# wangheda/youtube-8m

Measured on AMD Instinct MI355X. Metric: training videos/sec, higher is better.
Workload: dtype f32; 1 GPU; BASELINE configs[3]: LstmModel (2 x BasicLSTMCell(1024), dynamic_rnn over F=300) on raw uint8 [B,300,1152] frames + MoeModel head (2 mixtures, V=4716), fp32 training step (fwd+bwd+clip+Adam); per_gpu_batch=128, global_batch=128, frames=300, parallelism=dp1, params=113902808

## Files before the change

### include/yt8m_hip.h

```cpp
#ifndef YT8M_HIP_H
#define YT8M_HIP_H
#include <stdint.h>

#ifdef __cplusplus
extern "C" {
#endif

typedef void* yt8m_stream_t;

enum yt8m_status { YT8M_OK = 0, YT8M_E_BADARG = -1, YT8M_E_SHAPE = -2, YT8M_E_HIP = -3, YT8M_E_RCCL = -4 };
enum yt8m_label_dtype { YT8M_LABEL_U8 = 0, YT8M_LABEL_F32 = 1 };

int yt8m_abi_version(void);
const char* yt8m_last_error(void);
const char* yt8m_built_arch(void);

int yt8m_prof_enable(int on);
int yt8m_prof_reset(void);
int yt8m_prof_get(int family, int64_t* launches, double* total_ms);
int yt8m_prof_get_flops(int family, double* flops);
int yt8m_prof_get_bytes(int family, double* bytes);

int yt8m_probe_mfma_f32(int iters, int blocks, float* sink, yt8m_stream_t stream);
int yt8m_probe_mfma_bf16(int iters, int blocks, int random_operands, float* sink, yt8m_stream_t stream);
// ... 10 lines not shown
                          const float* A, int64_t lda, int64_t strideA, const float* B, int64_t ldb, int64_t strideB,
                          float* C, int64_t ldc, int64_t strideC, float beta, int64_t batch, yt8m_stream_t stream);

typedef struct yt8m_gemm_problem {
  int64_t M, N, K;
  const void* A; int64_t lda;
  const void* B; int64_t ldb;
  float* C; int64_t ldc;
  const float* bias;
  float beta;
} yt8m_gemm_problem;
int64_t yt8m_gemm_workspace_bytes(void);
int yt8m_gemm_f32_grouped(int transA, int transB, int nprob, const yt8m_gemm_problem* probs, void* workspace,
                          int64_t workspace_bytes, yt8m_stream_t stream);
int yt8m_gemm_bf16_nt_grouped(int nprob, const yt8m_gemm_problem* probs, void* workspace, int64_t workspace_bytes,
                              yt8m_stream_t stream);
int64_t yt8m_x3_image_bytes(int64_t rows, int64_t K);
int yt8m_x3_split(const float* src, int64_t R, int64_t C, int64_t ld, float scale, void* plain, void* trans, yt8m_stream_t stream);
int yt8m_gemm_x3_nt_grouped(int nprob, const yt8m_gemm_problem* probs, void* workspace, int64_t workspace_bytes,
                            yt8m_stream_t stream);
int yt8m_h2_split(const float* src, int64_t R, int64_t C, int64_t ld, float scale, const float* dscale, void* plain, void* trans,
                  float* colpart, yt8m_stream_t stream);
int yt8m_h2_absmax(const float* src, int64_t R, int64_t C, int64_t ld, void* word, yt8m_stream_t stream);
int yt8m_h2_degraded(uint64_t* counts, int reset, yt8m_stream_t stream);
int yt8m_h2_split_dropout(const float* src, int64_t R, int64_t C, float scale, const float* dscale, void* plain, void* trans,
                          float keep_prob, uint64_t seed, int64_t offset, yt8m_stream_t stream);
int yt8m_h2_split_rowmax(const float* src, int64_t R, int64_t C, int64_t ld, const void* rowmax, float* inv, void* plain,
                         yt8m_stream_t stream);
int yt8m_h2_split_ex(const float* src, int64_t R, int64_t C, int64_t ld, float scale, const void* dscale, const float* rowscale, void* plain,
                     void* trans, void* trans_scaled, float* colpart, float* colpart_scaled, yt8m_stream_t stream);
int yt8m_gemm_h1x2_nt_ex(int64_t M, int64_t N, int64_t K, const void* A1, int64_t ska, const void* B2, int64_t skb, float* C, int64_t ldc,
                         const float* bias, float alpha, const void* dsb, const float* rowscale, const float* colsum, float colsum_scale,
                         float beta, void* workspace, int64_t workspace_bytes, yt8m_stream_t stream);
int yt8m_h2_rowscales(const float* src, int64_t R, int64_t C, int64_t ld, float* S, float* inv, yt8m_stream_t stream);
int yt8m_h2_split_rows(const float* src, int64_t R, int64_t C, int64_t ld, const float* S, void* plain, yt8m_stream_t stream);
int yt8m_gemm_h2_nt_ex(int64_t M, int64_t N, int64_t K, const void* A2, int64_t ska, const void* B2, int64_t skb, float* C, int64_t ldc,
                       const float* bias, float alpha, const void* dsa, const void* dsb, const float* rowscale, float beta, void* workspace,
                       int64_t workspace_bytes, yt8m_stream_t stream);
int yt8m_timepool_max_f32(const float* y, int64_t F, int64_t B, int64_t N, int64_t ldy, float* out, int32_t* idx, int64_t ldo,
                          yt8m_stream_t stream);
int yt8m_timepool_shiftmax_f32(const float* z, int64_t F, int64_t B, int64_t ldz, int nfilt, const int32_t* fs, const int32_t* ncol, float* out,
                               int32_t* idx, int64_t ldo, yt8m_stream_t stream);
int yt8m_u8_cnn_pool_dw(const uint8_t* q, const float* r_tm, const int32_t* idx, const float* g, int64_t ldg, int64_t B, int64_t F, int64_t D,
                        int64_t N, int64_t fs, float* dW, float beta, yt8m_stream_t stream);
int yt8m_f32_cnn_pool_dw(const float* x, int64_t ldx, const int32_t* idx, const float* g, int64_t ldg, int64_t B, int64_t F, int64_t D,
                         int64_t N, int64_t fs, float* dW, int64_t lddw, float beta, yt8m_stream_t stream);
// ... 345 lines not shown
  int32_t input_u8;
  float forget_bias;
  int32_t fwd_chunks;
  int32_t bwd_chunks;
  int32_t need_dx;
  float input_keep_prob;
  int32_t reserved0;
  uint64_t dropout_seed[8];
} yt8m_lstm_stack_desc;
int yt8m_lstm_stack_supported(const yt8m_lstm_stack_desc* desc);
int64_t yt8m_lstm_stack_tape_bytes(const yt8m_lstm_stack_desc* desc);
int64_t yt8m_lstm_stack_scratch_bytes(const yt8m_lstm_stack_desc* desc);
int yt8m_lstm_stack_partition(const yt8m_lstm_stack_desc* desc, int* fwd_chunks, int* bwd_chunks);
int yt8m_lstm_stack_streams(int L, yt8m_stream_t* layer_streams, yt8m_stream_t* wgrad_stream);
int yt8m_lstm_stack_fwd(const yt8m_lstm_stack_desc* desc, const void* x, const int32_t* num_frames, const float* const* W,
                        const float* const* b, void* tape, int64_t tape_bytes, void* scratch, int64_t scratch_bytes,
                        yt8m_stream_t stream);
int yt8m_lstm_stack_view(const yt8m_lstm_stack_desc* desc, void* tape, int layer, int which, float** out);
int yt8m_lstm_stack_bwd(const yt8m_lstm_stack_desc* desc, const void* x, const int32_t* num_frames, const float* const* W, void* tape,
                        int64_t tape_bytes, void* scratch, int64_t scratch_bytes, const float* dout_top,
                        const float* const* dc_final, const float* const* dh_final, float* const* dW, float* const* db,
                        const float* beta_W, const float* beta_b, float* dx, yt8m_stream_t stream);
int yt8m_lstm_stack_status(const yt8m_lstm_stack_desc* desc, void* scratch, yt8m_stream_t stream);
int yt8m_lstm_stack_layer_done_wait(int layer, yt8m_stream_t stream);
int yt8m_lstm_stack_use_streams(int set, int* previous);
typedef void (*yt8m_stream_hook)(void* user, yt8m_stream_t stream);
int yt8m_lstm_stack_set_prep_hook(yt8m_stream_hook hook, void* user);
typedef struct yt8m_opt_ranges {
  float* w;
  float* m;
  float* v;
  const float* g;
  const int32_t* chunks;
  const int32_t* tensor_chunk_start;
  const int32_t* tensor_chunk_start_host;
  const float* l2;
  float* partial;
  float* norms;
  const uint8_t* skip_tensor;
  const yt8m_wimg_job* jobs;
  const int32_t* job_tensor_host;
  const int64_t* job_tile_base_host;
  int32_t njobs;
  int32_t nranges;
  int32_t range_lo[8], range_hi[8];
  float gscale, clip, lr_t, beta1, beta2, eps;
// ... 211 lines not shown
```

### youtube-8m_amd/_lib.py

```python
import ctypes
import os

_HERE = os.path.dirname(os.path.abspath(__file__))
LIB_PATH = os.environ.get("YT8M_LIB", os.path.join(_HERE, "libyt8m_hip.so"))

c_void_p, c_int, c_int64, c_float, c_double = ctypes.c_void_p, ctypes.c_int, ctypes.c_int64, ctypes.c_float, ctypes.c_double
P = c_void_p

class GemmProblem(ctypes.Structure):
    _fields_ = [("M", c_int64), ("N", c_int64), ("K", c_int64), ("A", c_void_p), ("lda", c_int64), ("B", c_void_p),
                ("ldb", c_int64), ("C", c_void_p), ("ldc", c_int64), ("bias", c_void_p), ("beta", c_float)]


STREAM_HOOK = ctypes.CFUNCTYPE(None, ctypes.c_void_p, ctypes.c_void_p)


class PersistBwdImages(ctypes.Structure):
    _fields_ = [("plain", ctypes.c_void_p), ("trans", ctypes.c_void_p), ("trans_scaled", ctypes.c_void_p), ("rowscale", ctypes.c_void_p),
                ("colpart", ctypes.c_void_p), ("colpart_scaled", ctypes.c_void_p)]


class LstmStackDesc(ctypes.Structure):
    _fields_ = [("B", c_int64), ("F", c_int64), ("D", c_int64), ("H", c_int64), ("L", ctypes.c_int32), ("input_u8", ctypes.c_int32),
                ("forget_bias", c_float), ("fwd_chunks", ctypes.c_int32), ("bwd_chunks", ctypes.c_int32), ("need_dx", ctypes.c_int32),
# ... 58 lines not shown
                                     c_int64, P]),
    "yt8m_bf16_image": (c_int, [P, c_int64, c_int64, c_int64, c_float, P, P, P]),
    "yt8m_gemm_b1_nt_grouped": (c_int, [c_int, ctypes.POINTER(GemmProblem), P, c_int64, P]),
    "yt8m_gemm_b1_nt_grouped_bf16c": (c_int, [c_int, ctypes.POINTER(GemmProblem), ctypes.c_uint, P, c_int64, P]),
    "yt8m_x3_split_ex": (c_int, [P, c_int64, c_int64, c_int64, c_float, P, P, P, P, P]),
    "yt8m_x3_split_colsum": (c_int, [P, c_int64, c_int64, c_int64, c_float, P, P, P, P, P, P, P]),
    "yt8m_x3_set_combine": (c_int, [c_int]),
    "yt8m_x3_set_schedule": (c_int, [c_int]),
    "yt8m_bf16_image_colsum": (c_int, [P, c_int64, c_int64, c_int64, c_float, P, P, P, P, P, P, P]),
    "yt8m_gemm_b1_nt_ex": (c_int, [c_int64, c_int64, c_int64, P, c_int64, P, c_int64, P, c_int64, P, c_float, P, P, c_float, c_float, P,
                                   c_int64, P]),
    "yt8m_u8_frames_image_t": (c_int, [P, P, c_int64, c_int64, c_int64, P, P]),
    "yt8m_lstm_stack_supported": (c_int, [DESC]),
    "yt8m_lstm_stack_tape_bytes": (c_int64, [DESC]),
    "yt8m_lstm_stack_scratch_bytes": (c_int64, [DESC]),
    "yt8m_lstm_stack_partition": (c_int, [DESC, ctypes.POINTER(c_int), ctypes.POINTER(c_int)]),
    "yt8m_lstm_stack_set_prep_hook": (c_int, [P, P]),
    "yt8m_lstm_stack_streams": (c_int, [c_int, PP, ctypes.POINTER(c_void_p)]),
    "yt8m_lstm_stack_fwd": (c_int, [DESC, P, P, PP, PP, P, c_int64, P, c_int64, P]),
    "yt8m_lstm_stack_view": (c_int, [DESC, P, c_int, c_int, ctypes.POINTER(c_void_p)]),
    "yt8m_lstm_stack_bwd": (c_int, [DESC, P, P, PP, P, c_int64, P, c_int64, P, PP, PP, PP, PP, ctypes.POINTER(c_float),
                                    ctypes.POINTER(c_float), P, P]),
    "yt8m_lstm_stack_status": (c_int, [DESC, P, P]),
    "yt8m_lstm_stack_layer_done_wait": (c_int, [c_int, P]),
    "yt8m_u8_frames_image": (c_int, [P, P, c_int64, c_int64, c_int64, c_float, P, P, P, P]),
    "yt8m_cast_f32_bf16": (c_int, [P, c_int64, c_int64, c_int64, P, c_int64, c_int, P]),
    "yt8m_cast_f32_bf16_dual": (c_int, [P, c_int64, c_int64, c_int64, P, c_int64, P, c_int64, P]),
    "yt8m_gemm_f32_batched": (c_int, [c_int, c_int, c_int64, c_int64, c_int64, P, c_int64, c_int64, P, c_int64, c_int64,
                                      P, c_int64, c_int64, c_float, c_int64, P]),
    "yt8m_l2norm_fwd_f32": (c_int, [P, P, c_int64, c_int64, c_float, P]),
    "yt8m_l2norm_bwd_f32": (c_int, [P, P, P, c_int64, c_int64, c_float, P]),
    "yt8m_dequant_l2norm_u8": (c_int, [P, P, P, c_int64, c_int64, c_int64, c_float, P]),
    "yt8m_dequant_mean_l2norm_u8": (c_int, [P, P, P, c_int64, c_int64, c_int64, c_float, P]),
    "yt8m_moe_workspace_bytes": (c_int64, [c_int64, c_int64]),
    "yt8m_moe_workspace_bytes_ex": (c_int64, [c_int64, c_int64, c_int64, c_int]),
    "yt8m_moe_fwd": (c_int, [P, P, P, P, P, c_int, c_int64, c_int64, c_int64, c_int, c_float, P, P, P, P, P, c_int64, P]),
    "yt8m_moe_bwd": (c_int, [P, P, P, P, P, P, c_int, c_int64, c_int64, c_int64, c_int, c_float, c_float, P, P, P, c_float, P, P,
                             c_int64, P]),
    "yt8m_logistic_fwd_bwd": (c_int, [P, P, P, P, c_int, c_int64, c_int64, c_int64, c_float, P, P, P, P, P, c_float, P, P,
                                      c_int64, P]),
    "yt8m_moe_mix_fwd": (c_int, [P, P, P, c_int64, c_int64, c_int, P]),
    "yt8m_moe_mix_bwd": (c_int, [P, P, P, c_int64, c_int64, c_int, P]),
    "yt8m_moe_mix_xent_workspace_bytes": (c_int64, [c_int64, c_int64]),
    "yt8m_moe_mix_xent_fwd": (c_int, [P, P, P, c_int, P, P, c_int64, c_int64, c_int, c_float, P, P]),
    "yt8m_moe_mix_xent_bwd": (c_int, [P, P, P, c_int, P, c_int64, c_int64, c_int, c_float, c_float, P]),
    "yt8m_moe_mix_xent_bwd_absmax": (c_int, [P, P, P, c_int, P, c_int64, c_int64, c_int, c_float, c_float, P, P]),
# ... 282 lines not shown
```

### youtube-8m_amd/csrc/gemm_x3.hip

```cpp
#include "common.h"
#include "x3_image.h"
#include "philox.h"
#include <type_traits>
#include <algorithm>
#include <mutex>
#include <stdlib.h>

namespace {

constexpr int TM = 256, TN = 256;
constexpr int PLANE_F = 256 * 8;
constexpr int OP_F = 3 * PLANE_F;
constexpr int NST = 3;
using yt8m_x3::RG_F;
using yt8m_x3::store_block;

typedef float f32x16 __attribute__((ext_vector_type(16)));
typedef __bf16 bf16x8 __attribute__((ext_vector_type(8)));

struct XArgs {
  const float* A;
  const float* B;
  float* C;
  const float* bias;
// ... 899 lines not shown
      v0.x += a0.x; v0.y += a0.y; v0.z += a0.z; v0.w += a0.w;
      v1.x += a1.x; v1.y += a1.y; v1.z += a1.z; v1.w += a1.w;
      v0.x += b0.x; v0.y += b0.y; v0.z += b0.z; v0.w += b0.w;
      v1.x += b1.x; v1.y += b1.y; v1.z += b1.z; v1.w += b1.w;
    }
    if (s < S) {
      const float4 a0 = *reinterpret_cast<const float4*>(base + (int64_t)s * pstride + e);
      const float4 a1 = *reinterpret_cast<const float4*>(base + (int64_t)s * pstride + e1);
      v0.x += a0.x; v0.y += a0.y; v0.z += a0.z; v0.w += a0.w;
      v1.x += a1.x; v1.y += a1.y; v1.z += a1.z; v1.w += a1.w;
    }
    finish_store(g, v0, m0 + e / TN, n0 + (e % TN));
    finish_store(g, v1, m0 + e1 / TN, n0 + (e1 % TN));
  }
}

template <int NP>
__global__ __launch_bounds__(256) void x3_split_kernel(const float* __restrict__ src, int64_t ld, int R, int Cc, float* __restrict__ plain,
                                                       float* __restrict__ trans, float scale, const float* __restrict__ rowscale,
                                                       float* __restrict__ trans_s, float* __restrict__ colpart = nullptr,
                                                       float* __restrict__ colpart_s = nullptr, const float* __restrict__ dscale = nullptr,
                                                       const float* __restrict__ rowS = nullptr, const unsigned* __restrict__ rowmaxw = nullptr,
                                                       float* __restrict__ rowinv = nullptr, unsigned long long* __restrict__ degraded = nullptr,
                                                       float drop_keep = 0.f, unsigned long long drop_seed = 0ull, long long drop_off = 0) {
  __shared__ float T[64][65];
  if (dscale) scale *= yt8m_x3::pow2_scale_for(__uint_as_float(reinterpret_cast<const unsigned*>(dscale)[0]), 14);
  const int r0 = blockIdx.y * 64, c0 = blockIdx.x * 64;
  const int t = threadIdx.x;
  unsigned n_clamp = 0, n_flush = 0;
  {
    const int c4 = (t & 15) * 4, rr = t >> 4;
    const bool vec = (ld & 3) == 0 && (reinterpret_cast<uintptr_t>(src) & 15) == 0;
#pragma unroll
    for (int i = 0; i < 4; ++i) {
      const int r = rr + 16 * i;
      float4 v = {0.f, 0.f, 0.f, 0.f};
      if (r0 + r < R) {
        const float* p = src + (int64_t)(r0 + r) * ld + c0 + c4;
        if (vec && c0 + c4 + 3 < Cc) v = *reinterpret_cast<const float4*>(p);
        else {
          if (c0 + c4 + 0 < Cc) v.x = p[0];
          if (c0 + c4 + 1 < Cc) v.y = p[1];
          if (c0 + c4 + 2 < Cc) v.z = p[2];
          if (c0 + c4 + 3 < Cc) v.w = p[3];
        }
      }
      if (drop_keep > 0.f && r0 + r < R) {
// ... 51 lines not shown
      if (weighted) {
        for (int r = 0; r < 64; ++r) acc += (r0 + r < R ? rowscale[r0 + r] : 0.f) * T[r][c];
      } else {
        for (int r = 0; r < 64; ++r) acc += T[r][c];
      }
      if constexpr (NP == 2) acc *= 1.0f / scale;
      dst[(int64_t)blockIdx.y * Cc + c0 + c] = acc;
    }
  }
  const int a = t & 63, blk = t >> 6;
  if (plain) {
    const int KB = (Cc + 15) >> 4;
    const int row = r0 + a, kb = (c0 >> 4) + blk;
    if (row < ((R + 31) & ~31) && kb < KB) {
      float v[16];
#pragma unroll
      for (int j = 0; j < 16; ++j) v[j] = T[a][blk * 16 + j];
      if constexpr (NP == 2) yt8m_x3::store_block_h2(v, plain + ((int64_t)(row >> 5) * KB + kb) * (NP * RG_F), row);
      else store_block<NP>(v, plain + ((int64_t)(row >> 5) * KB + kb) * (NP * RG_F), row);
    }
  }
  if (trans || trans_s) {
    const int KB = (R + 15) >> 4;
    const int row = c0 + a, kb = (r0 >> 4) + blk;
    if (row < ((Cc + 31) & ~31) && kb < KB) {
      float v[16];
#pragma unroll
      for (int j = 0; j < 16; ++j) v[j] = T[blk * 16 + j][a];
      if (trans) {
        if constexpr (NP == 2) yt8m_x3::store_block_h2(v, trans + ((int64_t)(row >> 5) * KB + kb) * (NP * RG_F), row);
        else store_block<NP>(v, trans + ((int64_t)(row >> 5) * KB + kb) * (NP * RG_F), row);
      }
      if (trans_s) {
#pragma unroll
        for (int j = 0; j < 16; ++j) {
          const int r = r0 + blk * 16 + j;
          v[j] *= r < R ? rowscale[r] : 0.f;
        }
        if constexpr (NP == 2) yt8m_x3::store_block_h2(v, trans_s + ((int64_t)(row >> 5) * KB + kb) * (NP * RG_F), row);
        else store_block<NP>(v, trans_s + ((int64_t)(row >> 5) * KB + kb) * (NP * RG_F), row);
      }
    }
  }
}

}

using namespace yt8m;

namespace {
constexpr size_t H2_DEGRADED_BYTES = 256 * 128;
unsigned long long* h2_degraded_words() {
  static std::mutex mu;
  static unsigned long long* words[64] = {};
  static bool tried[64] = {};
  int dev = 0;
  if (hipGetDevice(&dev) != hipSuccess || dev < 0 || dev >= 64) return nullptr;
  std::lock_guard<std::mutex> lk(mu);
  if (!tried[dev]) {
    tried[dev] = true;
    void* p = nullptr;
    if (hipMalloc(&p, H2_DEGRADED_BYTES) == hipSuccess && hipMemset(p, 0, H2_DEGRADED_BYTES) == hipSuccess) words[dev] = static_cast<unsigned long long*>(p);
    else (void)hipGetLastError();
// ... 70 lines not shown
  ProfScope prof(F_ELEMENTWISE, as_stream(stream));
  hipLaunchKernelGGL(x3_split_kernel<2>, grid, dim3(256), 0, as_stream(stream), src, ld, (int)R, (int)C, static_cast<float*>(plain),
                     static_cast<float*>(trans), scale, (const float*)nullptr, (float*)nullptr, colpart, (float*)nullptr, dscale,
                     (const float*)nullptr, (const unsigned*)nullptr, (float*)nullptr, h2_degraded_words());
  return launch_status("x3_split_kernel<2>");
}

extern "C" int yt8m_h2_split_dropout(const float* src, int64_t R, int64_t C, float scale, const float* dscale, void* plain, void* trans,
                                     float keep_prob, uint64_t seed, int64_t offset, yt8m_stream_t stream) {
  YT8M_REQUIRE(R >= 0 && C >= 0 && (plain || trans), YT8M_E_BADARG, "bad split arguments");
  YT8M_REQUIRE(keep_prob > 0.f && keep_prob <= 1.f && offset >= 0, YT8M_E_BADARG, "keep_prob in (0, 1], offset >= 0");
  YT8M_REQUIRE(R < (1LL << 31) && C < (1LL << 31), YT8M_E_BADARG, "matrix too large");
  YT8M_REQUIRE(((reinterpret_cast<uintptr_t>(plain) | reinterpret_cast<uintptr_t>(trans)) & 15) == 0, YT8M_E_BADARG,
               "images must be 16-byte aligned");
  if (R == 0 || C == 0) return YT8M_OK;
  dim3 grid((unsigned)((C + 63) / 64), (unsigned)((R + 63) / 64));
  YT8M_REQUIRE(grid.y < 65536, YT8M_E_BADARG, "too many rows for one split launch");
  ProfScope prof(F_ELEMENTWISE, as_stream(stream));
  hipLaunchKernelGGL(x3_split_kernel<2>, grid, dim3(256), 0, as_stream(stream), src, C, (int)R, (int)C, static_cast<float*>(plain),
                     static_cast<float*>(trans), scale, (const float*)nullptr, (float*)nullptr, (float*)nullptr, (float*)nullptr, dscale,
                     (const float*)nullptr, (const unsigned*)nullptr, (float*)nullptr, h2_degraded_words(),
                     keep_prob < 1.f ? keep_prob : 0.f, (unsigned long long)seed, (long long)offset);
  return launch_status("x3_split_kernel<2>");
}

extern "C" int yt8m_h2_split_ex(const float* src, int64_t R, int64_t C, int64_t ld, float scale, const void* dscale, const float* rowscale,
                                void* plain, void* trans, void* trans_scaled, float* colpart, float* colpart_scaled, yt8m_stream_t stream) {
  YT8M_REQUIRE(R >= 0 && C >= 0 && ld >= C && (plain || trans || trans_scaled), YT8M_E_BADARG, "bad split arguments");
  YT8M_REQUIRE((rowscale != nullptr) == (trans_scaled != nullptr || colpart_scaled != nullptr), YT8M_E_BADARG,
               "rowscale comes with trans_scaled / colpart_scaled");
  YT8M_REQUIRE(R < (1LL << 31) && C < (1LL << 31), YT8M_E_BADARG, "matrix too large");
  YT8M_REQUIRE(((reinterpret_cast<uintptr_t>(plain) | reinterpret_cast<uintptr_t>(trans) | reinterpret_cast<uintptr_t>(trans_scaled)) & 15) == 0,
               YT8M_E_BADARG, "images must be 16-byte aligned");
  if (R == 0 || C == 0) return YT8M_OK;
  dim3 grid((unsigned)((C + 63) / 64), (unsigned)((R + 63) / 64));
  YT8M_REQUIRE(grid.y < 65536, YT8M_E_BADARG, "too many rows for one split launch");
  ProfScope prof(F_ELEMENTWISE, as_stream(stream));
  hipLaunchKernelGGL(x3_split_kernel<2>, grid, dim3(256), 0, as_stream(stream), src, ld, (int)R, (int)C, static_cast<float*>(plain),
                     static_cast<float*>(trans), scale, rowscale, static_cast<float*>(trans_scaled), colpart, colpart_scaled,
                     static_cast<const float*>(dscale), (const float*)nullptr, (const unsigned*)nullptr, (float*)nullptr, h2_degraded_words());
  return launch_status("x3_split_kernel<2>");
}

namespace {
__global__ __launch_bounds__(256) void h2_absmax_kernel(const float* __restrict__ src, int64_t ld, int R, int Cc, unsigned* __restrict__ word) {
  __shared__ float red[4];
// ... 371 lines not shown
```

### youtube-8m_amd/csrc/lstm_stack.hip

```cpp
#include <stdlib.h>
#include <algorithm>
#include <mutex>
#include <vector>
#include "common.h"

using namespace yt8m;

namespace {

constexpr int MAXL = 8, MAXP = 64;
constexpr int MAXBP = 62;
constexpr float U8_ALPHA = 4.0f / 255.0f;
constexpr float U8_BETA = 128.0f * (4.0f / 255.0f) + (4.0f / 512.0f - 2.0f);
constexpr int64_t X3_MIN_ROWS = 1024;
constexpr int64_t STEP_IMAGES_MAX_BYTES = 8LL << 30;
constexpr float H2_S = 8192.0f;

int64_t up256(int64_t v) { return (v + 255) / 256 * 256; }

int knob(const char* name, int dflt) { const char* v = getenv(name); return v ? atoi(v) : dflt; }

struct Part { int64_t t0, T; };
int chunks(int64_t F, int n, Part* out) {
  if (n < 1) n = 1;
  if (n > F) n = (int)F;
  if (n > MAXP) n = MAXP;
  const int64_t step = (F + n - 1) / n;
  int k = 0;
  for (int64_t t0 = 0; t0 < F; t0 += step) out[k++] = {t0, std::min(step, F - t0)};
  return k;
}

struct Plan {
  int64_t B, F, D, H, FB;
  int L, u8, need_dx;
  int bf16;
  int nf, nb;
  Part fp[MAXP], bp[MAXP];
  int64_t z[MAXL], cs[MAXL], hs[MAXL], out[MAXL], rrow, tape_bytes;
  int64_t pws[MAXL], pws_bytes;
  int64_t gws[MAXL + 1], gws_bytes;
  int64_t gwx[MAXL], gws2;
  int64_t qimg, w3t, wcs, wxt3[MAXL], xi[MAXL];
  int64_t dz[MAXL], dbuf[MAXL], work[MAXL];
  int64_t dz3[MAXL], wx3[MAXL], dzT3[MAXL], dzT3s, csr, dbdummy;
  int64_t xT[MAXL], hT[MAXL];
  int64_t cpart[MAXL], cparts;
  bool colparts;
  int img_rows;
  int h2;
  int64_t hsc;
  int64_t hx0;
  int64_t hrow, hrow_stride;
  float keep;
  uint64_t seed[MAXL];
  int emit_max;
  int64_t rmax, rmax_stride;
  int64_t cimg[MAXL], cimgs;
  int64_t scratch_bytes;
};

int64_t x3_bytes(int64_t rows, int64_t K) { return yt8m_x3_image_bytes(rows, K); }
int64_t x1_bytes(int64_t rows, int64_t K) { return ((rows + 31) / 32) * ((K + 15) / 16) * 1024; }

const char* plan(const yt8m_lstm_stack_desc* d, Plan* P) {
  if (!d) return "null description";
  if (d->L < 1 || d->L > MAXL) return "1..8 layers";
  if (d->B < 1 || d->F < 1 || d->D < 1 || d->H < 1) return "empty dimension";
  Plan& p = *P;
// ... 46 lines not shown
    p.hs[l] = o; o += up256((FBH + BH) * 4);
    p.out[l] = o; o += up256(FBH * 4);
  }
  p.rrow = o; o += up256(p.FB * 4);
  p.tape_bytes = o;
  int64_t pb = yt8m_lstm_persist_workspace_bytes_steps(p.B, p.H, tmax);
  const bool per_step = pb <= STEP_IMAGES_MAX_BYTES;
  if (!per_step) pb = yt8m_lstm_persist_workspace_bytes(p.B, p.H);
  p.pws_bytes = up256(pb);
  o = 0;
  for (int l = 0; l < p.L; ++l) { p.pws[l] = o; o += p.pws_bytes; }
  p.gws_bytes = up256(yt8m_gemm_workspace_bytes());
  for (int l = 0; l <= p.L; ++l) { p.gws[l] = o; o += p.gws_bytes; }
  for (int l = 0; l < p.L; ++l) { p.gwx[l] = o; o += p.gws_bytes; }
  p.gws2 = o; o += p.gws_bytes;
  auto ib = [&](int64_t rows, int64_t K) { return p.bf16 ? x1_bytes(rows, K) : x3_bytes(rows, K); };
  const int64_t H4 = 4 * p.H;
  p.qimg = o; o += p.u8 ? up256(x1_bytes(p.FB, p.D)) : 0;
  p.w3t = o; o += p.u8 ? up256(ib(H4, p.D)) : 0;
  p.wcs = o; o += up256(H4 * 4);
  int64_t fmax = 0, bmax = 0;
  for (int c = 0; c < p.nf; ++c) fmax = std::max(fmax, p.fp[c].T * p.B);
  for (int c = 0; c < p.nb; ++c) bmax = std::max(bmax, p.bp[c].T * p.B);
  for (int l = 0; l < p.L; ++l) {
    const int64_t Din = l ? p.H : p.D;
    const bool x1 = l == 0 && p.u8;
    p.wxt3[l] = o; o += x1 ? 0 : up256(ib(H4, Din));
    p.xi[l] = o; o += x1 ? 0 : up256(ib(fmax, Din));
    p.dz[l] = o; o += up256(FBH * 4 * 4);
    p.dbuf[l] = o; o += l + 1 < p.L ? up256(FBH * 4) : 0;
    p.work[l] = o; o += up256(4 * BH * 4);
    const bool dxl = l > 0 || p.need_dx;
    p.dz3[l] = o; o += dxl ? up256(ib(bmax, H4)) : 0;
    p.wx3[l] = o; o += dxl ? up256(ib(Din, H4)) : 0;
    p.xT[l] = o; o += x1 ? up256(x1_bytes(p.D, p.FB)) : up256(ib(Din, p.FB));
    p.hT[l] = o; o += up256(ib(p.H, p.FB));
  }
  p.h2 = (knob("YT8M_STACK_H2", 1) && !p.bf16) ? 1 : 0;
  p.keep = (d->input_keep_prob > 0.f && d->input_keep_prob < 1.f) ? d->input_keep_prob : 0.f;
  for (int l = 0; l < MAXL; ++l) p.seed[l] = d->dropout_seed[l];
  if (d->input_keep_prob < 0.f || d->input_keep_prob > 1.f) return "input_keep_prob must be in [0, 1]";
  if (p.keep > 0.f && (p.u8 || !p.h2 || p.keep < 0.3f || (p.D % 4) != 0 || (p.H % 4) != 0))
    return "input dropout: float input, f16 product forms (YT8M_STACK_H2), keep_prob >= 0.3, D % 4 == 0";
  p.img_rows = (knob("YT8M_STACK_FUSED_IMAGES", 0) && !p.bf16 && !p.h2) ? yt8m_lstm_persist_bwd_images_rows(p.B, p.H) : 0;
  const int64_t trows = p.img_rows ? p.FB : bmax;
  for (int l = 0; l < p.L; ++l) { p.dzT3[l] = o; o += up256(ib(H4, trows)); }
  p.dzT3s = o; o += p.u8 ? up256(ib(H4, trows)) : 0;
  const int64_t ci = p.img_rows ? up256((int64_t)p.img_rows * MAXP * 2 * H4 * 4) : 0;
  for (int l = 0; l < p.L; ++l) { p.cimg[l] = o; o += ci; }
  p.cimgs = o; o += p.u8 ? ci : 0;
  p.csr = o; o += up256(H4 * 4);
  p.dbdummy = o; o += up256(H4 * 4);
  p.hsc = o; o += 256 * MAXL;
  p.hx0 = o; o += 256;
  p.hrow_stride = up256(bmax * 4);
  p.hrow = o; o += p.h2 ? p.hrow_stride * 2 * MAXL : 0;
  p.emit_max = (p.h2 && knob("YT8M_STACK_DZ_MAXIMA", 1) && yt8m_lstm_persist_bwd_images_rows(p.B, p.H) > 0 && per_step && p.nb <= 61) ? 1 : 0;
  p.rmax_stride = up256(p.FB * 4);
  p.rmax = o; o += p.emit_max ? p.rmax_stride * p.L : 0;
  p.colparts = knob("YT8M_STACK_COLPARTS", 1) != 0;
  for (int c = 0; c < p.nb; ++c) p.colparts = p.colparts && (p.bp[c].t0 * p.B) % 64 == 0 && (p.bp[c].T * p.B) % 64 == 0;
  const int64_t cp = p.colparts ? up256(((p.FB + 63) / 64) * H4 * 4) : 0;
  for (int l = 0; l < p.L; ++l) { p.cpart[l] = o; o += cp; }
  p.cparts = o; o += p.u8 ? cp : 0;
  p.scratch_bytes = o;
  return nullptr;
}

struct DevState {
  hipStream_t rs[MAXL] = {nullptr};
  hipStream_t dxs[MAXL] = {nullptr};
  hipStream_t sw = nullptr, sw2 = nullptr;
  int prio = 0;
  bool prio_known = false;
  std::vector<hipEvent_t> ev[2];
  size_t used[2] = {0, 0};
  hipEvent_t layer_done[MAXL] = {nullptr};
  int layers_done = 0;
};
std::mutex g_mu;
constexpr int NSETS = 2;
DevState g_dev[NSETS][16];
thread_local int g_set = 0;
thread_local yt8m_stream_hook g_prep_hook = nullptr;
thread_local void* g_prep_user = nullptr;
struct EarlyOpt {
  bool set = false;
  yt8m_opt_ranges o;
  std::vector<int32_t> tcs, job_tensor;
  std::vector<int64_t> tile_base;
};
thread_local EarlyOpt g_early;

int high_stream(DevState& S, hipStream_t* s) {
  if (*s) return YT8M_OK;
  if (!S.prio_known) {
    int least = 0, greatest = 0;
    YT8M_HIP_CHECK(hipDeviceGetStreamPriorityRange(&least, &greatest));
    S.prio = greatest;
    S.prio_known = true;
  }
  YT8M_HIP_CHECK(hipStreamCreateWithPriority(s, hipStreamNonBlocking, S.prio));
  return YT8M_OK;
// ... 102 lines not shown
extern "C" int yt8m_lstm_stack_layer_done_wait(int layer, yt8m_stream_t stream) {
  int dev = 0;
  YT8M_HIP_CHECK(hipGetDevice(&dev));
  YT8M_REQUIRE(dev >= 0 && dev < 16, YT8M_E_BADARG, "device index out of range");
  std::lock_guard<std::mutex> lk(g_mu);
  DevState& S = g_dev[g_set][dev];
  YT8M_REQUIRE(layer >= 0 && layer < S.layers_done && S.layer_done[layer], YT8M_E_BADARG,
               "no backward call on this device has recorded that layer");
  YT8M_HIP_CHECK(hipStreamWaitEvent(as_stream(stream), S.layer_done[layer], 0));
  return YT8M_OK;
}

extern "C" int yt8m_lstm_stack_status(const yt8m_lstm_stack_desc* desc, void* scratch, yt8m_stream_t stream) {
  Plan P;
  const char* why = plan(desc, &P);
  YT8M_REQUIRE(!why, YT8M_E_SHAPE, why ? why : "");
  YT8M_REQUIRE(scratch, YT8M_E_BADARG, "null scratch");
  int rc = YT8M_OK;
  for (int l = 0; l < P.L; ++l) {
    const int r = yt8m_lstm_persist_status(at<char>(scratch, P.pws[l]), stream);
    if (r != YT8M_OK) rc = r;
  }
  return rc;
}

extern "C" int yt8m_lstm_stack_set_prep_hook(yt8m_stream_hook hook, void* user) {
  g_prep_hook = hook;
  g_prep_user = user;
  return YT8M_OK;
}

extern "C" int yt8m_lstm_stack_set_early_optimizer(const yt8m_opt_ranges* opt) {
  g_early.set = false;
  if (!opt) return YT8M_OK;
  YT8M_REQUIRE(opt->nranges >= 1 && opt->nranges <= 8 && opt->tensor_chunk_start_host, YT8M_E_BADARG, "1..8 ranges + the host chunk starts");
  int hi = 0;
  for (int r = 0; r < opt->nranges; ++r) {
    YT8M_REQUIRE(opt->range_lo[r] >= 0 && opt->range_hi[r] >= opt->range_lo[r], YT8M_E_BADARG, "bad tensor range");
    hi = std::max(hi, (int)opt->range_hi[r]);
  }
  YT8M_REQUIRE(opt->njobs >= 0 && (opt->njobs == 0 || (opt->job_tensor_host && opt->job_tile_base_host)), YT8M_E_BADARG, "job tables");
  g_early.o = *opt;
  g_early.tcs.assign(opt->tensor_chunk_start_host, opt->tensor_chunk_start_host + hi + 1);
  g_early.o.tensor_chunk_start_host = g_early.tcs.data();
  g_early.job_tensor.clear();
  g_early.tile_base.clear();
// ... 178 lines not shown
  Ev ev(*S, 1);
  hipStream_t main = as_stream(stream), sw = S->sw;
  static const int dx_stream = knob("YT8M_STACK_DX_STREAM", 0), two_sw = knob("YT8M_STACK_SW2", 0);
  const int fuse_dz = P.h2 ? 0 : knob("YT8M_STACK_FUSE_DZ_SPLIT", 0);
  const int64_t B = P.B, D = P.D, H = P.H, H4 = 4 * H, BH = B * H, FB = P.FB;
  const int64_t KBtot = FB / 16;
  const bool bf = P.bf16 != 0;
  const int64_t KBB = bf ? 1024 : 3072;
  auto split = [&](const float* src, int64_t R, int64_t C, int64_t ld, float scale, void* plain, void* trans, hipStream_t st) {
    return bf ? yt8m_bf16_image(src, R, C, ld, scale, plain, trans, (yt8m_stream_t)st) : yt8m_x3_split(src, R, C, ld, scale, plain, trans, (yt8m_stream_t)st);
  };
  auto gemm = [&](int n, const yt8m_gemm_problem* pr, void* ws, int64_t wsb, hipStream_t st) {
    return bf ? yt8m_gemm_b1_nt_grouped(n, pr, ws, wsb, (yt8m_stream_t)st) : yt8m_gemm_x3_nt_grouped(n, pr, ws, wsb, (yt8m_stream_t)st);
  };
  hipEvent_t start = ev.record(main);
  ev.wait(sw, start);
  if (two_sw) ev.wait(S->sw2, start);
  for (int l = 0; l < P.L; ++l) { ev.wait(S->rs[l], start); if (dx_stream) ev.wait(S->dxs[l], start); }
  if (P.h2)
    for (int l = 0; l < P.L; ++l) {
      YT8M_HIP_CHECK(hipMemsetAsync(at<char>(scratch, P.hsc + 256 * l + 4), 0, 248, S->rs[l]));
      if (P.emit_max && l >= 1) YT8M_HIP_CHECK(hipMemsetAsync(at<char>(scratch, P.rmax + l * P.rmax_stride), 0, (size_t)FB * 4, S->rs[l]));
    }
  for (int l = 0; l < P.L; ++l) {
    if (!dW[l]) continue;
    if (l == 0 && P.u8) {
      if (P.h2) RC(yt8m_u8_frames_image_t_f16(static_cast<const uint8_t*>(x), num_frames, B, P.F, D, at<char>(scratch, P.xT[0]), sw));
      else RC(yt8m_u8_frames_image_t(static_cast<const uint8_t*>(x), num_frames, B, P.F, D, at<char>(scratch, P.xT[0]), sw));
    } else {
      const float* src = l ? at<float>(tape, P.out[l - 1]) : static_cast<const float*>(x);
      const int64_t Din = l ? H : D;
      if (P.h2 && P.keep > 0.f)
        RC(yt8m_h2_split_dropout(src, FB, Din, l ? H2_S : 1.0f, l ? nullptr : at<float>(scratch, P.hx0), nullptr, at<char>(scratch, P.xT[l]),
                                 P.keep, P.seed[l], 0, (yt8m_stream_t)sw));
      else if (P.h2 && l >= 1) RC(yt8m_h2_split(src, FB, Din, Din, H2_S, nullptr, nullptr, at<char>(scratch, P.xT[l]), nullptr, (yt8m_stream_t)sw));
      else if (P.h2) RC(yt8m_h2_split(src, FB, Din, Din, 1.0f, at<float>(scratch, P.hx0), nullptr, at<char>(scratch, P.xT[0]), nullptr, (yt8m_stream_t)sw));
      else RC(split(src, FB, Din, Din, 1.0f, nullptr, at<char>(scratch, P.xT[l]), sw));
    }
    if (P.h2) RC(yt8m_h2_split(at<float>(tape, P.hs[l]), FB, H, H, H2_S, nullptr, nullptr, at<char>(scratch, P.hT[l]), nullptr, (yt8m_stream_t)sw));
    else RC(split(at<float>(tape, P.hs[l]), FB, H, H, 1.0f, nullptr, at<char>(scratch, P.hT[l]), sw));
  }
  yt8m_stream_hook hook = g_prep_hook;
  void* hook_user = g_prep_user;
  g_prep_hook = nullptr;
  g_prep_user = nullptr;
  bool early = g_early.set;
  g_early.set = false;
  if (two_sw) ev.wait(S->sw2, ev.record(sw));
  int phase[MAXL];
  bool wx3_done[MAXL];
  const void* wx_img[MAXL] = {nullptr};
  hipEvent_t dzT_free[MAXL] = {nullptr};
  const bool fused_img = P.img_rows > 0 && !dx_stream && !fuse_dz;
  int64_t img_done_rows[MAXL] = {0};
  int img_launches[MAXL] = {0};
  for (int l = 0; l < P.L; ++l) {
    hipStream_t s = S->rs[l];
    float* work = at<float>(scratch, P.work[l]);
    const float* dh = dh_final ? dh_final[l] : nullptr;
    const float* dc = dc_final ? dc_final[l] : nullptr;
    if (dh) YT8M_HIP_CHECK(hipMemcpyAsync(work, dh, (size_t)BH * 4, hipMemcpyDeviceToDevice, s));
    else YT8M_HIP_CHECK(hipMemsetAsync(work, 0, (size_t)BH * 4, s));
    if (dc) YT8M_HIP_CHECK(hipMemcpyAsync(work + BH, dc, (size_t)BH * 4, hipMemcpyDeviceToDevice, s));
// ... 130 lines not shown
        yt8m_x3_set_combine(0);
        RC(grc);
        if (P.keep > 0.f) RC(yt8m_dropout_f32(dst, dst, M * Din, P.keep, P.seed[l], t0 * B * Din, (yt8m_stream_t)sx));
        dx_ev = ev.record(sx);
        if (c == 0 && j == 0) last.push_back(dx_ev);
        }
      }
      hipStream_t sw = (two_sw && l == 0) ? S->sw2 : S->sw;
      ev.wait(sw, rb);
      void* gw = at<char>(scratch, (two_sw && l == 0) ? P.gws2 : P.gws[P.L]);
      const float bW = first ? (beta_W ? beta_W[l] : 0.f) : 1.f;
      const bool lastpart = c == 0 && j == 0;
      if (dW[l]) {
        if (l == 0 && P.u8 && P.h2) {
          const float* rr = at<float>(tape, P.rrow) + t0 * B;
          float* word = at<float>(scratch, P.hsc) + 1 + c;
          if (!P.emit_max) RC(yt8m_h2_absmax(dzc, M, H4, H4, word, (yt8m_stream_t)sw));
          float* cp = P.colparts ? at<float>(scratch, P.cpart[l]) + (t0 * B / 64) * H4 : nullptr;
          float* cps = P.colparts ? at<float>(scratch, P.cparts) + (t0 * B / 64) * H4 : nullptr;
          RC(yt8m_h2_split_ex(dzc, M, H4, H4, 1.0f, word, rr, nullptr, at<char>(scratch, P.dzT3[l]), at<char>(scratch, P.dzT3s), cp, cps,
                              (yt8m_stream_t)sw));
          RC(yt8m_gemm_h1x2_nt_ex(D, H4, M, at<char>(scratch, P.xT[0]) + kb0 * 1024, KBtot, at<char>(scratch, P.dzT3s), 0, dW[0], H4, nullptr,
                                  U8_ALPHA, word, nullptr, nullptr, 0.f, bW, gw, P.gws_bytes, (yt8m_stream_t)sw));
          yt8m_gemm_problem pr = {H, H4, M, at<char>(scratch, P.hT[0]) + kb0 * 2048, KBtot, at<char>(scratch, P.dzT3[l]), 0,
                                  dW[0] + D * H4, H4, nullptr, bW};
          const float alpha = 1.0f / H2_S;
          const float* dsb = word;
          RC(yt8m_gemm_h2_nt_grouped(1, &pr, &alpha, nullptr, &dsb, gw, P.gws_bytes, (yt8m_stream_t)sw));
        } else if (l == 0 && P.u8) {
          const float* rr = at<float>(tape, P.rrow) + t0 * B;
          if (fused_img) {
          } else if (P.colparts || bf) {
            float* cp = P.colparts ? at<float>(scratch, P.cpart[l]) + (t0 * B / 64) * H4 : nullptr;
            float* cps = P.colparts ? at<float>(scratch, P.cparts) + (t0 * B / 64) * H4 : nullptr;
            if (bf) RC(yt8m_bf16_image_colsum(dzc, M, H4, H4, 1.0f, rr, nullptr, at<char>(scratch, P.dzT3[l]), at<char>(scratch, P.dzT3s), cp, cps, sw));
            else RC(yt8m_x3_split_colsum(dzc, M, H4, H4, 1.0f, rr, nullptr, at<char>(scratch, P.dzT3[l]), at<char>(scratch, P.dzT3s), cp, cps, sw));
          } else
            RC(yt8m_x3_split_ex(dzc, M, H4, H4, 1.0f, rr, nullptr, at<char>(scratch, P.dzT3[l]), at<char>(scratch, P.dzT3s), sw));
          if (bf)
            RC(yt8m_gemm_b1_nt_ex(D, H4, M, at<char>(scratch, P.xT[0]) + kb0 * 1024, KBtot, dzTs_img, 0, dW[0], H4,
                                  nullptr, U8_ALPHA, nullptr, nullptr, 0.f, bW, gw, P.gws_bytes, sw));
          else
            RC(yt8m_gemm_x1x3_nt_ex(D, H4, M, at<char>(scratch, P.xT[0]) + kb0 * 1024, KBtot, dzTs_img, 0, dW[0], H4,
                                    nullptr, U8_ALPHA, nullptr, nullptr, 0.f, bW, gw, P.gws_bytes, sw));
          yt8m_gemm_problem pr = {H, H4, M, at<char>(scratch, P.hT[0]) + kb0 * KBB, KBtot, dzT_img, 0,
                                  dW[0] + D * H4, H4, nullptr, bW};
          RC(gemm(1, &pr, gw, P.gws_bytes, sw));
        } else if (P.h2) {
          float* word = at<float>(scratch, P.hsc + 256 * l) + 1 + c;
          if (!P.emit_max) RC(yt8m_h2_absmax(dzc, M, H4, H4, word, (yt8m_stream_t)sw));
          float* cp = (P.colparts && db[l]) ? at<float>(scratch, P.cpart[l]) + (t0 * B / 64) * H4 : nullptr;
          RC(yt8m_h2_split(dzc, M, H4, H4, 1.0f, word, nullptr, at<char>(scratch, P.dzT3[l]), cp, (yt8m_stream_t)sw));
          yt8m_gemm_problem pr[2] = {
              {Din, H4, M, at<char>(scratch, P.xT[l]) + kb0 * 2048, KBtot, at<char>(scratch, P.dzT3[l]), 0, dW[l], H4, nullptr, bW},
              {H, H4, M, at<char>(scratch, P.hT[l]) + kb0 * 2048, KBtot, at<char>(scratch, P.dzT3[l]), 0, dW[l] + Din * H4, H4, nullptr, bW}};
          const float alphas[2] = {l ? 1.0f / H2_S : 1.0f, 1.0f / H2_S};
          const float* dsa[2] = {l ? nullptr : at<float>(scratch, P.hx0), nullptr};
          const float* dsb[2] = {word, word};
          RC(yt8m_gemm_h2_nt_grouped(2, pr, alphas, dsa, dsb, gw, P.gws_bytes, (yt8m_stream_t)sw));
        } else {
          if (fused_img) {
          } else if (!fused_t) {
            if (P.colparts && db[l]) {
              float* cp = at<float>(scratch, P.cpart[l]) + (t0 * B / 64) * H4;
              if (bf) RC(yt8m_bf16_image_colsum(dzc, M, H4, H4, 1.0f, nullptr, nullptr, at<char>(scratch, P.dzT3[l]), nullptr, cp, nullptr, sw));
              else RC(yt8m_x3_split_colsum(dzc, M, H4, H4, 1.0f, nullptr, nullptr, at<char>(scratch, P.dzT3[l]), nullptr, cp, nullptr, sw));
            } else {
              RC(split(dzc, M, H4, H4, 1.0f, nullptr, at<char>(scratch, P.dzT3[l]), sw));
            }
          }
          yt8m_gemm_problem pr[2] = {
              {Din, H4, M, at<char>(scratch, P.xT[l]) + kb0 * KBB, KBtot, dzT_img, 0, dW[l], H4, nullptr, bW},
              {H, H4, M, at<char>(scratch, P.hT[l]) + kb0 * KBB, KBtot, dzT_img, 0, dW[l] + Din * H4, H4, nullptr, bW}};
          RC(gemm(2, pr, gw, P.gws_bytes, sw));
          if (fused_t) dzT_free[l] = ev.record(sw);
        }
      }
      if (lastpart) {
        const float bb = beta_b ? beta_b[l] : 0.f;
        const int64_t ntile = (FB + 63) / 64;
        const int64_t nimg = (int64_t)img_launches[l] * P.img_rows;
        if (dW[l] && l == 0 && P.u8) {
          float* dbo = db[0] ? db[0] : at<float>(scratch, P.dbdummy);
          if (fused_img) {
            RC(yt8m_colsum_f32(at<float>(scratch, P.cimgs), nimg, H4, H4, at<float>(scratch, P.csr), 0.f, gw, P.gws_bytes, sw));
            if (db[0]) RC(yt8m_colsum_f32(at<float>(scratch, P.cimg[0]), nimg, H4, H4, db[0], bb, gw, P.gws_bytes, sw));
          } else if (P.colparts) {
            RC(yt8m_colsum_f32(at<float>(scratch, P.cparts), ntile, H4, H4, at<float>(scratch, P.csr), 0.f, gw, P.gws_bytes, sw));
            if (db[0]) RC(yt8m_colsum_f32(at<float>(scratch, P.cpart[0]), ntile, H4, H4, db[0], bb, gw, P.gws_bytes, sw));
          } else {
            RC(yt8m_colsum_weighted_f32(dz, FB, H4, H4, at<float>(tape, P.rrow), dbo, db[0] ? bb : 0.f, at<float>(scratch, P.csr), gw,
                                        P.gws_bytes, sw));
          }
          RC(yt8m_rank1_add_rows_f32(dW[0], D, H4, H4, at<float>(scratch, P.csr), U8_BETA, sw));
        } else if (db[l]) {
          if (fused_img) RC(yt8m_colsum_f32(at<float>(scratch, P.cimg[l]), nimg, H4, H4, db[l], bb, gw, P.gws_bytes, sw));
// ... 16 lines not shown
```

Baseline: 8312 videos/s.

## Alias lower layer's transposed h image onto upper layer's input image with leading block

For stacked LSTM backward, the transposed hidden-state image of layer l (h_{t-1} shifted) is now a view into layer l+1's transposed input image, which is laid out with a leading B-row pad so that both shifts share one buffer. This removes one split/transpose kernel and its scratch buffer per non-top layer. A new range-split entry point writes into the image at a custom K-block stride, and the weight-gradient GEMMs use the new strides and offsets. It relies on exact alignment of time shifts and zero-filled lead blocks, and is disabled under input dropout or when B is not a multiple of 16.

Measured after the change: 8357 videos/s (median of 6 runs). Within noise of the previous version (+0.6%).

```diff
diff --git a/include/yt8m_hip.h b/include/yt8m_hip.h
--- a/include/yt8m_hip.h
+++ b/include/yt8m_hip.h
@@ -56,6 +56,8 @@
 int yt8m_h2_split(const float* src, int64_t R, int64_t C, int64_t ld, float scale, const float* dscale, void* plain, void* trans,
                   float* colpart, yt8m_stream_t stream);
 int yt8m_h2_absmax(const float* src, int64_t R, int64_t C, int64_t ld, void* word, yt8m_stream_t stream);
+int yt8m_split_trans_range(int planes, const float* src, int64_t R, int64_t C, int64_t ld, float scale, const float* dscale, void* trans,
+                           int64_t trans_kb, yt8m_stream_t stream);
 int yt8m_h2_degraded(uint64_t* counts, int reset, yt8m_stream_t stream);
 int yt8m_h2_split_dropout(const float* src, int64_t R, int64_t C, float scale, const float* dscale, void* plain, void* trans,
                           float keep_prob, uint64_t seed, int64_t offset, yt8m_stream_t stream);
@@ -447,6 +449,7 @@
                         const float* const* dc_final, const float* const* dh_final, float* const* dW, float* const* db,
                         const float* beta_W, const float* beta_b, float* dx, yt8m_stream_t stream);
 int yt8m_lstm_stack_status(const yt8m_lstm_stack_desc* desc, void* scratch, yt8m_stream_t stream);
+int yt8m_lstm_stack_ht_views(int64_t* views, int reset);
 int yt8m_lstm_stack_layer_done_wait(int layer, yt8m_stream_t stream);
 int yt8m_lstm_stack_use_streams(int set, int* previous);
 typedef void (*yt8m_stream_hook)(void* user, yt8m_stream_t stream);
diff --git a/youtube-8m_amd/_lib.py b/youtube-8m_amd/_lib.py
--- a/youtube-8m_amd/_lib.py
+++ b/youtube-8m_amd/_lib.py
@@ -104,6 +104,8 @@
     "yt8m_lstm_stack_bwd": (c_int, [DESC, P, P, PP, P, c_int64, P, c_int64, P, PP, PP, PP, PP, ctypes.POINTER(c_float),
                                     ctypes.POINTER(c_float), P, P]),
     "yt8m_lstm_stack_status": (c_int, [DESC, P, P]),
+    "yt8m_lstm_stack_ht_views": (c_int, [ctypes.POINTER(c_int64), c_int]),
+    "yt8m_split_trans_range": (c_int, [c_int, P, c_int64, c_int64, c_int64, c_float, P, P, c_int64, P]),
     "yt8m_lstm_stack_layer_done_wait": (c_int, [c_int, P]),
     "yt8m_u8_frames_image": (c_int, [P, P, c_int64, c_int64, c_int64, c_float, P, P, P, P]),
     "yt8m_cast_f32_bf16": (c_int, [P, c_int64, c_int64, c_int64, P, c_int64, c_int, P]),
diff --git a/youtube-8m_amd/csrc/gemm_x3.hip b/youtube-8m_amd/csrc/gemm_x3.hip
--- a/youtube-8m_amd/csrc/gemm_x3.hip
+++ b/youtube-8m_amd/csrc/gemm_x3.hip
@@ -945,7 +945,8 @@
                                                        float* __restrict__ colpart_s = nullptr, const float* __restrict__ dscale = nullptr,
                                                        const float* __restrict__ rowS = nullptr, const unsigned* __restrict__ rowmaxw = nullptr,
                                                        float* __restrict__ rowinv = nullptr, unsigned long long* __restrict__ degraded = nullptr,
-                                                       float drop_keep = 0.f, unsigned long long drop_seed = 0ull, long long drop_off = 0) {
+                                                       float drop_keep = 0.f, unsigned long long drop_seed = 0ull, long long drop_off = 0,
+                                                       int trans_kb = 0) {
   __shared__ float T[64][65];
   if (dscale) scale *= yt8m_x3::pow2_scale_for(__uint_as_float(reinterpret_cast<const unsigned*>(dscale)[0]), 14);
   const int r0 = blockIdx.y * 64, c0 = blockIdx.x * 64;
@@ -1043,14 +1044,15 @@
   }
   if (trans || trans_s) {
     const int KB = (R + 15) >> 4;
+    const int KBs = trans_kb > 0 ? trans_kb : KB;
     const int row = c0 + a, kb = (r0 >> 4) + blk;
     if (row < ((Cc + 31) & ~31) && kb < KB) {
       float v[16];
 #pragma unroll
       for (int j = 0; j < 16; ++j) v[j] = T[blk * 16 + j][a];
       if (trans) {
-        if constexpr (NP == 2) yt8m_x3::store_block_h2(v, trans + ((int64_t)(row >> 5) * KB + kb) * (NP * RG_F), row);
-        else store_block<NP>(v, trans + ((int64_t)(row >> 5) * KB + kb) * (NP * RG_F), row);
+        if constexpr (NP == 2) yt8m_x3::store_block_h2(v, trans + ((int64_t)(row >> 5) * KBs + kb) * (NP * RG_F), row);
+        else store_block<NP>(v, trans + ((int64_t)(row >> 5) * KBs + kb) * (NP * RG_F), row);
       }
       if (trans_s) {
 #pragma unroll
@@ -1058,8 +1060,8 @@
           const int r = r0 + blk * 16 + j;
           v[j] *= r < R ? rowscale[r] : 0.f;
         }
-        if constexpr (NP == 2) yt8m_x3::store_block_h2(v, trans_s + ((int64_t)(row >> 5) * KB + kb) * (NP * RG_F), row);
-        else store_block<NP>(v, trans_s + ((int64_t)(row >> 5) * KB + kb) * (NP * RG_F), row);
+        if constexpr (NP == 2) yt8m_x3::store_block_h2(v, trans_s + ((int64_t)(row >> 5) * KBs + kb) * (NP * RG_F), row);
+        else store_block<NP>(v, trans_s + ((int64_t)(row >> 5) * KBs + kb) * (NP * RG_F), row);
       }
     }
   }
@@ -1176,6 +1178,28 @@
                      (const float*)nullptr, (const unsigned*)nullptr, (float*)nullptr, h2_degraded_words(),
                      keep_prob < 1.f ? keep_prob : 0.f, (unsigned long long)seed, (long long)offset);
   return launch_status("x3_split_kernel<2>");
+}
+
+extern "C" int yt8m_split_trans_range(int planes, const float* src, int64_t R, int64_t C, int64_t ld, float scale, const float* dscale,
+                                      void* trans, int64_t trans_kb, yt8m_stream_t stream) {
+  YT8M_REQUIRE(planes >= 1 && planes <= 3 && R >= 0 && C >= 0 && ld >= C && trans, YT8M_E_BADARG, "bad split arguments");
+  YT8M_REQUIRE(R < (1LL << 31) && C < (1LL << 31) && trans_kb >= (R + 15) / 16 && trans_kb < (1LL << 31), YT8M_E_BADARG,
+               "matrix too large or a K-block stride below the range");
+  YT8M_REQUIRE(planes == 2 || !dscale, YT8M_E_BADARG, "a device scale word comes with the h2 form only");
+  YT8M_REQUIRE((reinterpret_cast<uintptr_t>(trans) & 15) == 0, YT8M_E_BADARG, "images must be 16-byte aligned");
+  if (R == 0 || C == 0) return YT8M_OK;
+  dim3 grid((unsigned)((C + 63) / 64), (unsigned)((R + 63) / 64));
+  YT8M_REQUIRE(grid.y < 65536, YT8M_E_BADARG, "too many rows for one split launch");
+  ProfScope prof(F_ELEMENTWISE, as_stream(stream));
+  const auto launch = [&](auto kernel, unsigned long long* degraded) {
+    hipLaunchKernelGGL(kernel, grid, dim3(256), 0, as_stream(stream), src, ld, (int)R, (int)C, (float*)nullptr, static_cast<float*>(trans),
+                       scale, (const float*)nullptr, (float*)nullptr, (float*)nullptr, (float*)nullptr, dscale, (const float*)nullptr,
+                       (const unsigned*)nullptr, (float*)nullptr, degraded, 0.f, 0ull, 0ll, (int)trans_kb);
+  };
+  if (planes == 3) launch(x3_split_kernel<3>, nullptr);
+  else if (planes == 2) launch(x3_split_kernel<2>, h2_degraded_words());
+  else launch(x3_split_kernel<1>, nullptr);
+  return launch_status(planes == 2 ? "x3_split_kernel<2>" : "x3_split_kernel");
 }
 
 extern "C" int yt8m_h2_split_ex(const float* src, int64_t R, int64_t C, int64_t ld, float scale, const void* dscale, const float* rowscale,
diff --git a/youtube-8m_amd/csrc/lstm_stack.hip b/youtube-8m_amd/csrc/lstm_stack.hip
--- a/youtube-8m_amd/csrc/lstm_stack.hip
+++ b/youtube-8m_amd/csrc/lstm_stack.hip
@@ -45,6 +45,9 @@
   int64_t dz[MAXL], dbuf[MAXL], work[MAXL];
   int64_t dz3[MAXL], wx3[MAXL], dzT3[MAXL], dzT3s, csr, dbdummy;
   int64_t xT[MAXL], hT[MAXL];
+  int64_t xT_kb[MAXL], hT_kb[MAXL];
+  int64_t xT_lead[MAXL];
+  int ht_view[MAXL];
   int64_t cpart[MAXL], cparts;
   bool colparts;
   int img_rows;
@@ -137,6 +140,7 @@
   int64_t fmax = 0, bmax = 0;
   for (int c = 0; c < p.nf; ++c) fmax = std::max(fmax, p.fp[c].T * p.B);
   for (int c = 0; c < p.nb; ++c) bmax = std::max(bmax, p.bp[c].T * p.B);
+  const bool ht_views = p.B % 16 == 0 && !(d->input_keep_prob > 0.f && d->input_keep_prob < 1.f);
   for (int l = 0; l < p.L; ++l) {
     const int64_t Din = l ? p.H : p.D;
     const bool x1 = l == 0 && p.u8;
@@ -148,9 +152,15 @@
     const bool dxl = l > 0 || p.need_dx;
     p.dz3[l] = o; o += dxl ? up256(ib(bmax, H4)) : 0;
     p.wx3[l] = o; o += dxl ? up256(ib(Din, H4)) : 0;
-    p.xT[l] = o; o += x1 ? up256(x1_bytes(p.D, p.FB)) : up256(ib(Din, p.FB));
-    p.hT[l] = o; o += up256(ib(p.H, p.FB));
-  }
+    const bool lead = l >= 1 && ht_views;
+    p.xT_lead[l] = lead ? p.B / 16 : 0;
+    p.xT_kb[l] = p.FB / 16 + p.xT_lead[l];
+    p.xT[l] = o; o += x1 ? up256(x1_bytes(p.D, p.FB)) : up256(ib(Din, p.FB + 16 * p.xT_lead[l]));
+    p.ht_view[l] = (l + 1 < p.L && ht_views) ? 1 : 0;
+    p.hT_kb[l] = p.FB / 16 + (p.ht_view[l] ? p.B / 16 : 0);
+    p.hT[l] = o; o += p.ht_view[l] ? 0 : up256(ib(p.H, p.FB));
+  }
+  for (int l = 0; l + 1 < p.L; ++l) if (p.ht_view[l]) p.hT[l] = p.xT[l + 1];
   p.h2 = (knob("YT8M_STACK_H2", 1) && !p.bf16) ? 1 : 0;
   p.keep = (d->input_keep_prob > 0.f && d->input_keep_prob < 1.f) ? d->input_keep_prob : 0.f;
   for (int l = 0; l < MAXL; ++l) p.seed[l] = d->dropout_seed[l];
@@ -194,6 +204,7 @@
   int layers_done = 0;
 };
 std::mutex g_mu;
+int64_t g_ht_views[16];
 constexpr int NSETS = 2;
 DevState g_dev[NSETS][16];
 thread_local int g_set = 0;
@@ -342,6 +353,16 @@
     if (r != YT8M_OK) rc = r;
   }
   return rc;
+}
+
+extern "C" int yt8m_lstm_stack_ht_views(int64_t* views, int reset) {
+  int dev = 0;
+  YT8M_HIP_CHECK(hipGetDevice(&dev));
+  YT8M_REQUIRE(dev >= 0 && dev < 16 && views, YT8M_E_BADARG, "device index out of range or NULL output");
+  std::lock_guard<std::mutex> lk(g_mu);
+  *views = g_ht_views[dev];
+  if (reset) g_ht_views[dev] = 0;
+  return YT8M_OK;
 }
 
 extern "C" int yt8m_lstm_stack_set_prep_hook(yt8m_stream_hook hook, void* user) {
@@ -566,23 +587,35 @@
       YT8M_HIP_CHECK(hipMemsetAsync(at<char>(scratch, P.hsc + 256 * l + 4), 0, 248, S->rs[l]));
       if (P.emit_max && l >= 1) YT8M_HIP_CHECK(hipMemsetAsync(at<char>(scratch, P.rmax + l * P.rmax_stride), 0, (size_t)FB * 4, S->rs[l]));
     }
+  int64_t views = 0;
   for (int l = 0; l < P.L; ++l) {
+    if (dW[l] || (l >= 1 && P.ht_view[l - 1] && dW[l - 1])) {
+      if (l == 0 && P.u8) {
+        if (P.h2) RC(yt8m_u8_frames_image_t_f16(static_cast<const uint8_t*>(x), num_frames, B, P.F, D, at<char>(scratch, P.xT[0]), sw));
+        else RC(yt8m_u8_frames_image_t(static_cast<const uint8_t*>(x), num_frames, B, P.F, D, at<char>(scratch, P.xT[0]), sw));
+      } else {
+        const float* src = l ? at<float>(tape, P.out[l - 1]) : static_cast<const float*>(x);
+        const int64_t Din = l ? H : D;
+        if (P.xT_lead[l])
+          RC(yt8m_split_trans_range(bf ? 1 : P.h2 ? 2 : 3, src, FB, Din, Din, P.h2 ? H2_S : 1.0f, nullptr,
+                                    at<char>(scratch, P.xT[l]) + P.xT_lead[l] * (P.h2 ? 2048 : KBB), P.xT_kb[l], (yt8m_stream_t)sw));
+        else if (P.h2 && P.keep > 0.f)
+          RC(yt8m_h2_split_dropout(src, FB, Din, l ? H2_S : 1.0f, l ? nullptr : at<float>(scratch, P.hx0), nullptr, at<char>(scratch, P.xT[l]),
+                                   P.keep, P.seed[l], 0, (yt8m_stream_t)sw));
+        else if (P.h2 && l >= 1) RC(yt8m_h2_split(src, FB, Din, Din, H2_S, nullptr, nullptr, at<char>(scratch, P.xT[l]), nullptr, (yt8m_stream_t)sw));
+        else if (P.h2) RC(yt8m_h2_split(src, FB, Din, Din, 1.0f, at<float>(scratch, P.hx0), nullptr, at<char>(scratch, P.xT[0]), nullptr, (yt8m_stream_t)sw));
+        else RC(split(src, FB, Din, Din, 1.0f, nullptr, at<char>(scratch, P.xT[l]), sw));
+      }
+    }
     if (!dW[l]) continue;
-    if (l == 0 && P.u8) {
-      if (P.h2) RC(yt8m_u8_frames_image_t_f16(static_cast<const uint8_t*>(x), num_frames, B, P.F, D, at<char>(scratch, P.xT[0]), sw));
-      else RC(yt8m_u8_frames_image_t(static_cast<const uint8_t*>(x), num_frames, B, P.F, D, at<char>(scratch, P.xT[0]), sw));
-    } else {
-      const float* src = l ? at<float>(tape, P.out[l - 1]) : static_cast<const float*>(x);
-      const int64_t Din = l ? H : D;
-      if (P.h2 && P.keep > 0.f)
-        RC(yt8m_h2_split_dropout(src, FB, Din, l ? H2_S : 1.0f, l ? nullptr : at<float>(scratch, P.hx0), nullptr, at<char>(scratch, P.xT[l]),
-                                 P.keep, P.seed[l], 0, (yt8m_stream_t)sw));
-      else if (P.h2 && l >= 1) RC(yt8m_h2_split(src, FB, Din, Din, H2_S, nullptr, nullptr, at<char>(scratch, P.xT[l]), nullptr, (yt8m_stream_t)sw));
-      else if (P.h2) RC(yt8m_h2_split(src, FB, Din, Din, 1.0f, at<float>(scratch, P.hx0), nullptr, at<char>(scratch, P.xT[0]), nullptr, (yt8m_stream_t)sw));
-      else RC(split(src, FB, Din, Din, 1.0f, nullptr, at<char>(scratch, P.xT[l]), sw));
-    }
+    if (P.ht_view[l]) { ++views; continue; }
     if (P.h2) RC(yt8m_h2_split(at<float>(tape, P.hs[l]), FB, H, H, H2_S, nullptr, nullptr, at<char>(scratch, P.hT[l]), nullptr, (yt8m_stream_t)sw));
     else RC(split(at<float>(tape, P.hs[l]), FB, H, H, 1.0f, nullptr, at<char>(scratch, P.hT[l]), sw));
+  }
+  if (views) {
+    int dev = 0;
+    YT8M_HIP_CHECK(hipGetDevice(&dev));
+    if (dev >= 0 && dev < 16) g_ht_views[dev] += views;
   }
   yt8m_stream_hook hook = g_prep_hook;
   void* hook_user = g_prep_user;
@@ -759,7 +792,7 @@
                               (yt8m_stream_t)sw));
           RC(yt8m_gemm_h1x2_nt_ex(D, H4, M, at<char>(scratch, P.xT[0]) + kb0 * 1024, KBtot, at<char>(scratch, P.dzT3s), 0, dW[0], H4, nullptr,
                                   U8_ALPHA, word, nullptr, nullptr, 0.f, bW, gw, P.gws_bytes, (yt8m_stream_t)sw));
-          yt8m_gemm_problem pr = {H, H4, M, at<char>(scratch, P.hT[0]) + kb0 * 2048, KBtot, at<char>(scratch, P.dzT3[l]), 0,
+          yt8m_gemm_problem pr = {H, H4, M, at<char>(scratch, P.hT[0]) + kb0 * 2048, P.hT_kb[0], at<char>(scratch, P.dzT3[l]), 0,
                                   dW[0] + D * H4, H4, nullptr, bW};
           const float alpha = 1.0f / H2_S;
           const float* dsb = word;
@@ -780,7 +813,7 @@
           else
             RC(yt8m_gemm_x1x3_nt_ex(D, H4, M, at<char>(scratch, P.xT[0]) + kb0 * 1024, KBtot, dzTs_img, 0, dW[0], H4,
                                     nullptr, U8_ALPHA, nullptr, nullptr, 0.f, bW, gw, P.gws_bytes, sw));
-          yt8m_gemm_problem pr = {H, H4, M, at<char>(scratch, P.hT[0]) + kb0 * KBB, KBtot, dzT_img, 0,
+          yt8m_gemm_problem pr = {H, H4, M, at<char>(scratch, P.hT[0]) + kb0 * KBB, P.hT_kb[0], dzT_img, 0,
                                   dW[0] + D * H4, H4, nullptr, bW};
           RC(gemm(1, &pr, gw, P.gws_bytes, sw));
         } else if (P.h2) {
@@ -789,8 +822,8 @@
           float* cp = (P.colparts && db[l]) ? at<float>(scratch, P.cpart[l]) + (t0 * B / 64) * H4 : nullptr;
           RC(yt8m_h2_split(dzc, M, H4, H4, 1.0f, word, nullptr, at<char>(scratch, P.dzT3[l]), cp, (yt8m_stream_t)sw));
           yt8m_gemm_problem pr[2] = {
-              {Din, H4, M, at<char>(scratch, P.xT[l]) + kb0 * 2048, KBtot, at<char>(scratch, P.dzT3[l]), 0, dW[l], H4, nullptr, bW},
-              {H, H4, M, at<char>(scratch, P.hT[l]) + kb0 * 2048, KBtot, at<char>(scratch, P.dzT3[l]), 0, dW[l] + Din * H4, H4, nullptr, bW}};
+              {Din, H4, M, at<char>(scratch, P.xT[l]) + (P.xT_lead[l] + kb0) * 2048, P.xT_kb[l], at<char>(scratch, P.dzT3[l]), 0, dW[l], H4, nullptr, bW},
+              {H, H4, M, at<char>(scratch, P.hT[l]) + kb0 * 2048, P.hT_kb[l], at<char>(scratch, P.dzT3[l]), 0, dW[l] + Din * H4, H4, nullptr, bW}};
           const float alphas[2] = {l ? 1.0f / H2_S : 1.0f, 1.0f / H2_S};
           const float* dsa[2] = {l ? nullptr : at<float>(scratch, P.hx0), nullptr};
           const float* dsb[2] = {word, word};
@@ -807,8 +840,8 @@
             }
           }
           yt8m_gemm_problem pr[2] = {
-              {Din, H4, M, at<char>(scratch, P.xT[l]) + kb0 * KBB, KBtot, dzT_img, 0, dW[l], H4, nullptr, bW},
-              {H, H4, M, at<char>(scratch, P.hT[l]) + kb0 * KBB, KBtot, dzT_img, 0, dW[l] + Din * H4, H4, nullptr, bW}};
+              {Din, H4, M, at<char>(scratch, P.xT[l]) + (P.xT_lead[l] + kb0) * KBB, P.xT_kb[l], dzT_img, 0, dW[l], H4, nullptr, bW},
+              {H, H4, M, at<char>(scratch, P.hT[l]) + kb0 * KBB, P.hT_kb[l], dzT_img, 0, dW[l] + Din * H4, H4, nullptr, bW}};
           RC(gemm(2, pr, gw, P.gws_bytes, sw));
           if (fused_t) dzT_free[l] = ev.record(sw);
         }
```
